# adjerbetian/OpenCL_PathTracer

Hardware: AMD Instinct MI355X
Metric: Msamples/s (paths x bounces) at 1920x1080 (higher is better)
Workload: dtype f32; 1 GPU; BASELINE configs[2]: synthetic random-triangle scene (numpy MT19937 seed 12345): 1000000 triangles (665533 BVH nodes, depth 22), 1920x1080, ray depth 10, JITTERED, 1 light(s); spp_total=256, parallelism=single GPU

## Files before the change

### opencl_pathtracer_amd/csrc/kernel_wavefront.hip

```cpp
#include <hip/hip_runtime.h>

#include "ptmi_device.hpp"
#include "ptmi_shading.hpp"
#include "ptmi_literal_path.hpp"

#include <atomic>
#include <cstdlib>
#include <cstring>

namespace PTMI_DEV_NS {

constexpr int kWfBlock = 256;
constexpr int kWfBlockNarrow = 64;
constexpr int kWfStack = PTMI_BVH_MAX_DEPTH;
#ifndef PTMI_WF_MIN_WAVES
#define PTMI_WF_MIN_WAVES 5
#endif
#ifndef PTMI_WF_MIN_WAVES_GENERAL
#define PTMI_WF_MIN_WAVES_GENERAL 5
#endif
#ifndef PTMI_WF_QUEUES
#define PTMI_WF_QUEUES 8
#endif
constexpr int kQueues = PTMI_WF_QUEUES;
// ... 20 lines not shown
    const DShade* shade;
    const DMat* mats;
    const ptmi_light* lights;
    const ptmi_texture* textures;
    const ptmi_uchar4* texels;
    uint32_t root_ref;
    uint32_t width, height;
    uint32_t max_depth, n_lights, sampler, tris_precomputed;
    uint32_t histograms;
    uint32_t boxes_ordered;
    uint32_t wide_records;
    uint32_t russian_roulette;
    uint32_t source_seed;
    uint32_t wait_debt;
    uint32_t split_paths;
};

constexpr uint32_t kStatDepthBins = 64;
constexpr uint32_t kPoisonMarker = 0x7FC0DEADu;
constexpr uint32_t kGivenUp = 0x80000000u, kGiveUpListFirst = (uint32_t)(kQueues * kQueueStride), kGiveUpListCap = 8u * 1024u - kGiveUpListFirst;
static_assert(kQueues * kQueueStride <= 1024, "the give-up list lies behind the queue counters inside the set's 8 x 1024 dwords");
constexpr uint32_t kSplitWords = C_TRI + 1;
static_assert(PTMI_COUNTER_SPLITS * (int)kSplitWords <= 64, "flushed by one wave");
__device__ __forceinline__ uint32_t counter_split_of(uint32_t slot, uint32_t split_paths)
{
    const uint32_t t1 = split_paths ? split_paths : 0xFFFFFFFFu, t2 = split_paths ? 2u * split_paths : 0xFFFFFFFFu,
                   t3 = split_paths ? 3u * split_paths : 0xFFFFFFFFu;
    return (slot >= t1 ? 1u : 0u) + (slot >= t2 ? 1u : 0u) + (slot >= t3 ? 1u : 0u);
}

// ... 24 lines not shown
    atomicAdd(&totals[C_SEGMENTS], (unsigned long long)n_seg - 1ull);
    atomicAdd(&totals[C_HITS], (unsigned long long)depth);
    atomicAdd(&totals[C_SHADOW], (unsigned long long)n_shadow);
    atomicAdd(&totals[C_BBX], (unsigned long long)pc.bbx);
    atomicAdd(&totals[C_TRI], (unsigned long long)pc.tri);
}

__device__ __forceinline__ void give_path_up(V4& radiance, V4& transfer, uint32_t& reflection, uint32_t& p_bbx, uint32_t& p_tri)
{
    const float m = __uint_as_float(kPoisonMarker);
    radiance = v4(m, m, m, m);
    transfer = v4(1, 1, 1, 1);
    reflection = 0; p_bbx = 0; p_tri = 0;
}

template <bool STATS, bool PRE, bool SS, bool PLAIN = false, bool NANSAFE = false, int BLOCK = 256>
__global__ void __launch_bounds__(BLOCK, PLAIN ? PTMI_WF_MIN_WAVES : PTMI_WF_MIN_WAVES_GENERAL) render_wavefront_kernel(
                                                                    const DScene* __restrict__ scene_in_memory, const DWarm sc_arg, const uint32_t first_iteration,
                                                                    const uint32_t n_iterations, const uint32_t iteration_stride,
                                                                    const uint32_t n_jobs,
                                                                    uint32_t* __restrict__ job_counter,
                                                                    const uint32_t stack_levels,
                                                                    float* __restrict__ stage,
                                                                    uint32_t* __restrict__ stage_stats)
{
    DWarm sc = sc_arg;
    if (PLAIN) { sc.sampler = PTMI_SAMPLER_JITTERED; sc.russian_roulette = 0; sc.n_lights = 1; }
    constexpr bool kOneLight = PLAIN;
    constexpr int kWfBlock = BLOCK;
    constexpr bool kTos = !PLAIN;
    extern __shared__ __attribute__((aligned(16))) uint32_t stack_mem[];
    constexpr uint32_t kBlockCounters = STATS ? (uint32_t)C_COUNT : PTMI_COUNTER_SPLITS * kSplitWords;
    static_assert(kBlockCounters <= 64, "zeroed and flushed by one wave");
    __shared__ unsigned long long block_counters[kBlockCounters];

    const uint32_t tid = threadIdx.x;
    if (tid < kBlockCounters) block_counters[tid] = 0;
    __syncthreads();
    uint32_t* const stack_floor = &stack_mem[kHitRecordWords * kWfBlock + tid];
    *stack_floor = REF_NONE;
    auto cold_scene = [&]() -> const DScene& {
        const DScene* p = scene_in_memory;
        asm volatile("" : "+s"(p));
        return *p;
    };
// ... 75 lines not shown
        cur = sc.root_ref; sp = stack_floor; tri_i = tri_end = 0;
        if (kTos) tos = REF_NONE;
        if (shadow) atomicAnd(&hit_mem[kWordTri * kWfBlock], ~kHitFound);
        else hit_mem[kWordTri * kWfBlock] = 0;
        exact_boxes = !(sc.boxes_ordered && ray_slabs_are_ordered(r));
        if (cur & REF_LEAF) {
            decode_leaf(sc, cur, tri_i, tri_end);
            cur = REF_NONE;
        }
    };

    unsigned long long* const key_mem = reinterpret_cast<unsigned long long*>(&stack_mem[(kHitRecordWords + 1 + stack_levels) * kWfBlock]);
    uint2* const item_mem = reinterpret_cast<uint2*>(&stack_mem[(kHitRecordWords + 3 + stack_levels) * kWfBlock]) + (tid & ~63u);
    const uint32_t lane = tid & 63u, wave_first = (uint32_t)__builtin_amdgcn_readfirstlane((int)(tid & ~63u));
    uint32_t pass_rounds = 0, pass_items = 0, item_violations = 0;
    const uint32_t n_records = STATS ? cold_scene().n_records : 0u;
    auto leaf_pass = [&](bool waits_at_leaf) {
        auto lanes_below = [&](unsigned long long m) {
            return __builtin_amdgcn_mbcnt_hi((uint32_t)(m >> 32), __builtin_amdgcn_mbcnt_lo((uint32_t)m, 0u));
        };
        const uint32_t left = tri_end - tri_i;
        const uint32_t offered = waits_at_leaf ? (left < 4u ? left : 4u) : 0u;
        const unsigned long long plane0 = __builtin_amdgcn_ballot_w64((offered & 1u) != 0), plane1 = __builtin_amdgcn_ballot_w64((offered & 2u) != 0),
                                 plane2 = __builtin_amdgcn_ballot_w64((offered & 4u) != 0);
        const int n_items = __popcll(plane0) + 2 * __popcll(plane1) + 4 * __popcll(plane2);
        const uint32_t first_item = lanes_below(plane0) + 2u * lanes_below(plane1) + 4u * lanes_below(plane2);
        const uint32_t room = first_item < 64u ? 64u - first_item : 0u;
        const uint32_t cnt = offered < room ? offered : room;
        const uint32_t n_now = n_items < 64 ? (uint32_t)n_items : 64u;
        if (STATS) { pass_rounds++; pass_items += n_now; }
// ... 63 lines not shown
                decode_leaf(sc, cur, tri_i, tri_end);
                cur = kTos ? tos : *sp;
                uint32_t* const under = sp - kWfBlock;
                sp = under < stack_floor ? stack_floor : under;
                if (kTos) tos = *sp;
            }
        }
    };
    auto node_step = [&]() {
        const float4* const rec = reinterpret_cast<const float4*>(&sc.tris[cur & REF_INDEX_MASK_INNER]);
        const float4 a = rec[0], b = rec[1], c = rec[2], d = rec[3];
        const float lo1[3] = {a.x, a.y, a.z}, hi1[3] = {a.w, b.x, b.y};
        const float lo2[3] = {b.z, b.w, c.x}, hi2[3] = {c.y, c.z, c.w};
        const uint32_t ref1 = __float_as_uint(d.x), ref2 = __float_as_uint(d.y), axis = __float_as_uint(d.z);
        const bool fwd = ((dir_signs >> axis) & 1u) != 0;
        bool h1, h2;
        if (!wave_exact) {
            h1 = box_hit_ordered(lo1, hi1, r, limit);
            h2 = box_hit_ordered(lo2, hi2, r, limit);
        } else {
            h1 = box_hit(lo1, hi1, (ref1 & REF_EMPTY) != 0, r, limit);
            h2 = box_hit(lo2, hi2, (ref2 & REF_EMPTY) != 0, r, limit);
        }
        p_bbx += 2;
        if (kTos) {
            const uint32_t far_ref = fwd ? ref2 : ref1;
            sp[kWfBlock] = far_ref;
            uint32_t* const pushed = sp + kWfBlock;
            const uint32_t child = fwd ? (h1 ? ref1 : ref2) : (h2 ? ref2 : ref1);
            cur = h1 ? child : (h2 ? child : tos);
            tos = h1 ? (h2 ? far_ref : tos) : tos;
            sp = h1 ? (h2 ? pushed : sp) : sp;
            if (!(h1 | h2)) {
                uint32_t* const below = sp - kWfBlock;
                sp = below < stack_floor ? stack_floor : below;
                tos = *sp;
            }
            if (cur != REF_NONE && (cur & REF_LEAF)) {
                decode_leaf(sc, cur, tri_i, tri_end);
                cur = tos;
                uint32_t* const under = sp - kWfBlock;
                sp = under < stack_floor ? stack_floor : under;
                tos = *sp;
            }
            return;
        }
        sp[kWfBlock] = fwd ? ref2 : ref1;
        uint32_t* const pushed = sp + kWfBlock;
        sp = h1 ? (h2 ? pushed : sp) : sp;
        const uint32_t popped = *sp;
        uint32_t* const below = sp - kWfBlock;
        uint32_t* const under = below < stack_floor ? stack_floor : below;
        const uint32_t child = fwd ? (h1 ? ref1 : ref2) : (h2 ? ref2 : ref1);
        cur = h1 ? child : (h2 ? child : popped);
        sp = h1 ? sp : (h2 ? sp : under);
        if (cur != REF_NONE && (cur & REF_LEAF)) {
            decode_leaf(sc, cur, tri_i, tri_end);
            cur = *sp;
            uint32_t* const under = sp - kWfBlock;
            sp = under < stack_floor ? stack_floor : under;
        }
    };

    int wait_debt = 0;
    bool pending, want_inner, want_post;
    int n_t, n_i, n_p;
    bool any_lane;
    unsigned long long dead_lanes = 0ull;
    auto survey = [&]() {
        pending = tri_i < tri_end;
        const bool has_node = cur < REF_DEAD;
        const unsigned long long b_t = __builtin_amdgcn_ballot_w64(pending), b_n = __builtin_amdgcn_ballot_w64(has_node), b_dead = dead_lanes;
        const unsigned long long m_t = b_t, m_i = b_n & ~b_t, m_p = ~(b_t | b_n | b_dead);
        want_inner = !pending & has_node;
        want_post = !pending & !has_node & (cur != REF_DEAD);
// ... 175 lines not shown
                }
                if (skip) {
                    if (owns_pixel) cold_scene().stage_flag[gy * sc.width + gx] = 0.f;
                    need_path = true;
                } else
                if (sc.max_depth > 0) {
                    limit = INFINITY;
                    new_ray = true;
                } else {
                    finish_path(false);
                }
            }
            if (new_ray) {
                ray_set_direction(r, new_direction);
                dir_signs = (r.d.x > 0 ? 1u : 0u) | (r.d.y > 0 ? 2u : 0u) | (r.d.z > 0 ? 4u : 0u);
                const float o_size = __builtin_fabsf(r.o.x) + __builtin_fabsf(r.o.y) + __builtin_fabsf(r.o.z) + __builtin_fabsf(r.o.w);
                const float d_size = __builtin_fabsf(r.d.x) + __builtin_fabsf(r.d.y) + __builtin_fabsf(r.d.z) + __builtin_fabsf(r.d.w);
                bool bad = !((o_size <= 0x1p+40f) & (d_size <= 4.0f));
                if (!PLAIN && !owns_pixel && __builtin_expect(bad, 0)) {
                    const uint32_t place = atomicAdd(&job_counter[2], 1u);
                    bad = place < kGiveUpListCap;
                    if (bad) {
                        job_counter[kGiveUpListFirst + place] = slot;
                        slot |= kGivenUp;
                    }
                }
                if (__builtin_expect(bad, 0)) {
                    give_path_up(radiance, transfer, reflection, p_bbx, p_tri);
                    shadow = false;
                    job_counter[1] = 1u;
// ... 6 lines not shown
        dead_lanes = __builtin_amdgcn_ballot_w64(cur == REF_DEAD);
        wave_exact = __builtin_amdgcn_ballot_w64(exact_boxes) != 0ull;
        if (STATS) cycles_p += __builtin_amdgcn_s_memtime() - pass_start;
    }

    if (STATS && (tid & 63u) == 0) {
        atomicAdd(&block_counters[C_TRIPS_I], (unsigned long long)trips_i);
        atomicAdd(&block_counters[C_LANES_I], lanes_i);
        atomicAdd(&block_counters[C_TRIPS_T], (unsigned long long)(pass_rounds));
        atomicAdd(&block_counters[C_LANES_T], (unsigned long long)pass_items);
        atomicAdd(&block_counters[C_TRIPS_P], (unsigned long long)trips_p);
        atomicAdd(&block_counters[C_LANES_P], lanes_p);
        atomicAdd(&block_counters[C_CYCLES_P], cycles_p);
        atomicAdd(&block_counters[C_CYCLES_LOOP], __builtin_amdgcn_s_memtime() - loop_start);
    }
    if (STATS && item_violations != 0u) atomicAdd(&block_counters[C_ITEM_VIOLATIONS], (unsigned long long)item_violations);
    __syncthreads();
    if (tid < (STATS ? 1u : (uint32_t)PTMI_COUNTER_SPLITS)) {
        unsigned long long* const totals = &block_counters[tid * kSplitWords];
        totals[C_SHADOW] = totals[C_HITS] * sc.n_lights;
    }
    __syncthreads();
    if (STATS) {
        if (tid < C_COUNT) atomicAdd(&cold_scene().counters[tid], block_counters[tid]);
    } else if (tid < kBlockCounters) {
        const uint32_t k = tid / kSplitWords, c = tid % kSplitWords;
        if (k == 0u || block_counters[tid] != 0ull) atomicAdd(&cold_scene().counters[k * C_COUNT + c], block_counters[tid]);
    }
}

// ... 235 lines not shown

static bool five_wide_workgroups_fit(const WavefrontLaunch& w)
{
    static std::atomic<int> wide_fits[kMaxCachedDevices][PTMI_BVH_MAX_DEPTH + 1];
    int fits = w.cached_device ? wide_fits[w.device][w.lv].load(std::memory_order_relaxed) : 0;
    if (fits == 0) {
        int n_cu = 0;
        const int wide = resident_blocks_of(PTMI_DEV_NS::render_wavefront_kernel<false, true, false, true, false>, w.lv, PTMI_DEV_NS::kWfBlock);
        const bool known = hipDeviceGetAttribute(&n_cu, hipDeviceAttributeMultiprocessorCount, w.device) == hipSuccess && n_cu > 0 && wide > 0;
        fits = known && wide < 5 * n_cu ? 2 : 1;
        if (w.cached_device) wide_fits[w.device][w.lv].store(fits, std::memory_order_relaxed);
    }
    return fits == 1;
}

template <bool S, bool P, bool A, bool L, bool N, int B>
static void launch_instance(const WavefrontLaunch& w)
{
    auto kernel = PTMI_DEV_NS::render_wavefront_kernel<S, P, A, L, N, B>;
    static std::atomic<int> resident_cache[kMaxCachedDevices][PTMI_BVH_MAX_DEPTH + 1];
    int resident = w.cached_device ? resident_cache[w.device][w.lv].load(std::memory_order_relaxed) : 0;
    if (resident == 0) {
        resident = resident_blocks_of(kernel, w.lv, B);
        if (w.cached_device) resident_cache[w.device][w.lv].store(resident, std::memory_order_relaxed);
    }
    if (w.cached_device) g_last_grid[w.device].store((uint32_t)B << 20 | (uint32_t)resident, std::memory_order_relaxed);
    uint32_t nb = (w.n_jobs + B - 1) / B;
    if (resident > 0 && nb > (uint32_t)resident) nb = (uint32_t)resident;
    hipLaunchKernelGGL(kernel, dim3(nb), dim3(B), wavefront_lds_bytes(w.lv, B), w.st, w.scene_in_device_memory, w.warm, w.first_iteration,
                       w.n_iterations, w.iteration_stride, w.n_jobs, w.job_counter, w.lv, w.stage, w.stage_stats);
}

using LaunchInstance = void (*)(const WavefrontLaunch&);
static LaunchInstance instance_for(const DScene& sc, bool scheduler_stats, bool plain, bool narrow)
{
    constexpr int kWide = PTMI_DEV_NS::kWfBlock, kNarrow = PTMI_DEV_NS::kWfBlockNarrow;
    const bool pre = sc.tris_precomputed != 0;
    if (sc.super_sampling) return pre ? launch_instance<true, true, true, false, true, kWide> : launch_instance<true, false, true, false, true, kWide>;
    if (scheduler_stats) return pre ? launch_instance<true, true, false, false, true, kWide> : launch_instance<true, false, false, false, true, kWide>;
    if (sc.nan_safe) {
        if (plain) return launch_instance<false, true, false, true, true, kWide>;
        return pre ? launch_instance<false, true, false, false, true, kWide> : launch_instance<false, false, false, false, true, kWide>;
    }
    if (plain)
        return narrow ? launch_instance<false, true, false, true, false, kNarrow> : launch_instance<false, true, false, true, false, kWide>;
    if (pre) return narrow ? launch_instance<false, true, false, false, false, kNarrow> : launch_instance<false, true, false, false, false, kWide>;
    return launch_instance<false, false, false, false, false, kWide>;
}

}

int PTMI_ARITH(launch_render_wavefront)(const DScene& sc, const DScene* scene_in_device_memory, uint32_t first_iteration,
                            uint32_t n_iterations, uint32_t iteration_stride, uint32_t* job_counter, uint32_t stack_levels,
                            bool scheduler_stats, float* stage, uint32_t* stage_stats, void* stream, std::string* err)
{
    if (n_iterations == 0) return PTMI_OK;
    const uint32_t tiles = ((sc.width + 7u) / 8u) * ((sc.height + 7u) / 8u);
    const uint64_t jobs64 = (uint64_t)tiles * 64u * n_iterations;
    if (jobs64 > (sc.sampler == PTMI_SAMPLER_RANDOM ? 0x7FFFFFF0ull : 0xFFFFFFF0ull)) {
        if (err) *err = "too many jobs in one launch";
        return PTMI_ERR_INVALID_ARGUMENT;
// ... 12 lines not shown
        w.first_iteration = first_iteration; w.n_iterations = n_iterations; w.iteration_stride = iteration_stride;
        w.job_counter = job_counter; w.stage = stage; w.stage_stats = stage_stats;
        w.cached_device = hipGetDevice(&w.device) == hipSuccess && w.device >= 0 && w.device < kMaxCachedDevices;
        const uint32_t lv = w.lv;
        PTMI_DEV_NS::DWarm& warm = w.warm;
        warm.nodes = sc.nodes; warm.tris = sc.tris; warm.big_leaves = sc.big_leaves; warm.tri_ids = sc.tri_ids; warm.shade = sc.shade;
        warm.mats = sc.mats; warm.lights = sc.lights; warm.textures = sc.textures; warm.texels = sc.texels;
        warm.root_ref = sc.root_ref; warm.width = sc.width; warm.height = sc.height; warm.max_depth = sc.max_depth;
        warm.n_lights = sc.n_lights; warm.sampler = sc.sampler; warm.tris_precomputed = sc.tris_precomputed;
        warm.histograms = sc.hist_depths != nullptr;
        warm.boxes_ordered = sc.boxes_ordered;
        warm.wide_records = sc.wide_records;
        warm.russian_roulette = sc.russian_roulette;
        warm.source_seed = sc.source_seed;
        warm.split_paths = sc.split_paths;
        const bool plain = sc.tris_precomputed && sc.plain_shading && sc.sampler == PTMI_SAMPLER_JITTERED && !sc.russian_roulette &&
                           sc.n_lights == 1 && !sc.super_sampling && !scheduler_stats;
        warm.wait_debt = lv >= 16u ? 768u : (plain ? 320u : 512u);
        const bool narrow = !five_wide_workgroups_fit(w) && std::getenv("PTMI_WIDE_WORKGROUPS") == nullptr;
        instance_for(sc, scheduler_stats, plain, narrow)(w);
        e = hipGetLastError();
        const dim3 redo_block(PTMI_DEV_NS::kBlock);
        if (e == hipSuccess && stage == nullptr && sc.sampler == PTMI_SAMPLER_RANDOM) {
            const auto redo_random = sc.tris_precomputed ? PTMI_DEV_NS::redo_random_kernel<true> : PTMI_DEV_NS::redo_random_kernel<false>;
            hipLaunchKernelGGL(redo_random, dim3(64), redo_block, 0, w.st, sc, first_iteration, n_iterations, iteration_stride, job_counter);
            e = hipGetLastError();
        }
        if (e == hipSuccess && stage != nullptr) {
            const auto redo_poisoned = sc.tris_precomputed ? PTMI_DEV_NS::redo_poisoned_kernel<true> : PTMI_DEV_NS::redo_poisoned_kernel<false>;
            hipLaunchKernelGGL(redo_poisoned, dim3(1024), redo_block, 0, w.st, sc, first_iteration, n_iterations, iteration_stride, stage,
// ... 36 lines not shown
```

### opencl_pathtracer_amd/csrc/ptmi_api.cpp

```cpp
#include <cstdlib>
#include <cstring>
#include <mutex>

#include "ptmi_context.h"

using namespace ptmi_internal;

namespace {
std::mutex g_err_mutex;
std::string g_err;
}

void ptmi_internal::set_global_error(const std::string& msg)
{
    std::lock_guard<std::mutex> lock(g_err_mutex);
    g_err = msg;
}

extern "C" {

int ptmi_abi_version(void) { return PTMI_ABI_VERSION; }

int ptmi_device_count(void)
{
// ... 57 lines not shown
        return fail(nullptr, PTMI_ERR_HIP, msg);
    }
    {
        const uint64_t tiles = (uint64_t)((cfg->image_width + 7u) / 8u) * ((cfg->image_height + 7u) / 8u);
        const uint64_t by_jobs = (cfg->sampler == PTMI_SAMPLER_RANDOM ? 0x7FFFFFF0ull : 0xFFFFFFF0ull) / (tiles * 64u);
        const uint64_t by_bytes = (4ull << 30) / ((uint64_t)cfg->image_width * cfg->image_height * 20u);
        uint64_t cap = kMaxIterationsPerLaunch;
        if (by_jobs < cap) cap = by_jobs;
        if (by_bytes < cap) cap = by_bytes;
        ctx->iterations_per_launch = cap < 1 ? 1u : (uint32_t)cap;
        if (const char* v = std::getenv("PTMI_ITERATIONS_PER_LAUNCH")) {
            const long want = std::strtol(v, nullptr, 10);
            if (want >= 1 && want <= 32 && (uint32_t)want < ctx->iterations_per_launch) ctx->iterations_per_launch = (uint32_t)want;
        }
    }
    *out = ctx;
    return PTMI_OK;
}

int ptmi_set_stream(ptmi_ctx* ctx, void* hip_stream)
{
    if (!ctx) return PTMI_ERR_INVALID_ARGUMENT;
    if (ctx->n_dev() != 1) return fail(ctx, PTMI_ERR_UNSUPPORTED, "ptmi_set_stream on a multi-device context");
    DeviceState& d = ctx->dev[0];
    ON_DEVICE(ctx, d);
    HIP_TRY(ctx, hipStreamSynchronize(d.stream));
    if (int rc = fold_events(ctx, d)) return rc;
    d.stream = hip_stream ? (hipStream_t)hip_stream : d.own_stream;
    return PTMI_OK;
}
// ... 186 lines not shown
```

### opencl_pathtracer_amd/csrc/ptmi_context.h

```cpp
#pragma once

#include <hip/hip_runtime.h>

#include <string>
#include <utility>
#include <vector>

#include "ptmi.h"
#include "ptmi_internal.h"
#include "scene_refit.h"
#include "launch_schedule.h"
#include "snapshot_ring.h"

namespace ptmi_internal {

struct DeviceScene {
    std::vector<void*> allocations;
    float* d_color = nullptr;
    float* d_count = nullptr;
    uint32_t* d_hist = nullptr;
    unsigned long long* d_counters = nullptr;
    uint32_t* d_job_counter = nullptr;
    DScene ds{};
    DScene* d_scene = nullptr;
// ... 36 lines not shown
    UpdateFacts update;
    RefitSchedule refit;
    bool have_refit = false;
    float* d_reduced = nullptr;
    uint8_t* d_display = nullptr;
    size_t display_bytes = 0;
};

}

struct ptmi_ctx : ptmi_internal::ContextScene {
    ptmi_config cfg{};
    std::vector<ptmi_internal::DeviceState> dev;
    std::string err;
    uint32_t iterations_per_launch = ptmi_internal::kMaxIterationsPerLaunch;
    std::vector<void*> rccl_comms;
    int rccl_state = 0;
    float* h_staging = nullptr;
    struct HostRange { char* p; size_t bytes; };
    std::vector<HostRange> pinned_host;
    char* d_query = nullptr;
    char* h_query = nullptr;
    size_t query_cap = 0;

    ptmi_internal::ContextScene& scene() { return *this; }
    uint32_t n_dev() const { return (uint32_t)dev.size(); }
    size_t npix() const { return (size_t)cfg.image_width * cfg.image_height; }
    size_t color_bytes() const { return npix() * 16; }
    size_t count_bytes() const { return npix() * 4; }
    size_t image_bytes() const { return npix() * 20; }
// ... 72 lines not shown
```

### opencl_pathtracer_amd/csrc/ptmi_internal.h

```cpp
#pragma once

#include <cstdint>
#include <string>

#include "ptmi.h"
#ifdef __HIPCC__
#include <hip/hip_runtime.h>
#endif

namespace ptmi_internal {

void set_global_error(const std::string& msg);

#ifdef __HIPCC__
inline int launch_status(hipError_t e, const char* kernel, std::string* err)
{
    if (e == hipSuccess) return PTMI_OK;
    if (err) *err = std::string(kernel) + " launch: " + hipGetErrorString(e);
    return PTMI_ERR_HIP;
}
#endif

constexpr uint32_t REF_LEAF = 0x80000000u;
constexpr uint32_t REF_EMPTY = 0x40000000u;
// ... 89 lines not shown
    uint32_t root_ref;
    uint32_t width, height;
    uint32_t max_depth;
    uint32_t n_lights;
    uint32_t sampler;
    uint32_t super_sampling;
    uint32_t tris_precomputed;
    uint32_t plain_shading;
    uint32_t nan_safe;
    uint32_t nan_walk_box_tests, nan_walk_tri_tests, nan_walk_last_tri;
    uint32_t n_records;
    uint32_t wide_records;
    uint32_t boxes_ordered;
    uint32_t russian_roulette;
    uint32_t source_seed;
};

#define PTMI_DECLARE_INTEGRATOR_ENTRY_POINTS(SUFFIX)                                                                             \
                                       \
    int launch_render##SUFFIX(const DScene& sc, uint32_t first_iteration, uint32_t n_iterations, uint32_t iteration_stride,      \
                              void* stream, std::string* err);                                                                  \
                            \
      \
    int launch_render_wavefront##SUFFIX(const DScene& sc, const DScene* scene_in_device_memory, uint32_t first_iteration,        \
                                        uint32_t n_iterations, uint32_t iteration_stride, uint32_t* job_counter,                \
                                        uint32_t stack_levels, bool scheduler_stats, float* stage,                              \
                                        uint32_t* stage_stats, void* stream, std::string* err);                                 \
    void last_wavefront_grid##SUFFIX(int device, uint32_t* lanes_per_workgroup, uint32_t* resident_workgroups);                  \
           \
    int launch_accumulate_staged##SUFFIX(const DScene& sc, uint32_t first_iteration, uint32_t n_iterations, const float* stage,  \
// ... 26 lines not shown
```

### opencl_pathtracer_amd/csrc/ptmi_scene_memory.cpp

```cpp
#include <algorithm>
#include <chrono>
#include <cstdlib>
#include <cstring>

#include "ptmi_context.h"
#include "scene_layout.h"

using namespace ptmi_internal;

bool ptmi_internal::one_path_per_lane(const ptmi_ctx* ctx)
{
    if ((ctx->cfg.flags & PTMI_FLAG_MEGAKERNEL) != 0) return true;
    if (ctx->literal_kernel_reason.empty()) return false;
    const char* force = std::getenv("PTMI_LITERAL_KERNEL");
    return ctx->cfg.sampler == PTMI_SAMPLER_RANDOM || (force && force[0] == '1');
}

int ptmi_internal::quiesce(ptmi_ctx* ctx, DeviceState& d)
{
    ON_DEVICE(ctx, d);
    d.schedule.forget();
    for (int i = 0; i < kStageSets; i++)
        if (d.launch_stream[i]) HIP_TRY(ctx, hipStreamSynchronize(d.launch_stream[i]));
    HIP_TRY(ctx, hipStreamSynchronize(d.stream));
// ... 128 lines not shown
        if (int rc = scene_alloc(ctx, d, ctx->count_bytes(), ds.stage_flag)) return rc;
        HIP_TRY(ctx, hipMemcpy(dx, kX2inv, sizeof kX2inv, hipMemcpyHostToDevice));
        ds.x2inv = dx;
    }
    ds.sky = *sc->sky;
    std::memcpy(ds.cam_pos, &sc->camera_position, 16);
    std::memcpy(ds.cam_dir, &sc->camera_direction, 16);
    std::memcpy(ds.cam_right, &sc->camera_right, 16);
    std::memcpy(ds.cam_up, &sc->camera_up, 16);
    ds.tris_precomputed = lay.tris_precomputed ? 1u : 0u;
    ds.plain_shading = lay.plain_shading ? 1u : 0u;
    ds.nan_safe = lay.literal_kernel_reason.empty() ? 0u : 1u;
    ds.nan_walk_box_tests = lay.nan_walk_box_tests; ds.nan_walk_tri_tests = lay.nan_walk_tri_tests; ds.nan_walk_last_tri = lay.nan_walk_last_tri;
    if (std::getenv("PTMI_WALK_NAN_RAYS") != nullptr) ds.nan_walk_box_tests = ds.nan_walk_tri_tests = 0xFFFFFFFFu;
    ds.boxes_ordered = (lay.boxes_ordered && std::getenv("PTMI_GENERIC_BOXES") == nullptr) ? 1u : 0u;
    ds.root_ref = lay.root_ref;
    ds.width = ctx->cfg.image_width;
    ds.height = ctx->cfg.image_height;
    ds.max_depth = ctx->cfg.ray_max_depth;
    ds.n_lights = ctx->cfg.lights_size;
    ds.sampler = ctx->cfg.sampler;
    ds.russian_roulette = (ctx->cfg.flags & PTMI_FLAG_RUSSIAN_ROULETTE) ? 1u : 0u;
    ds.source_seed = (ctx->cfg.flags & PTMI_FLAG_SOURCE_SEED) ? 1u : 0u;
    return upload_scene_records(ctx, d);
}

}

extern "C" {

// ... 254 lines not shown
```

### opencl_pathtracer_amd/csrc/scene_layout.cpp

```cpp
#include "scene_layout.h"
#include "scene_refit_common.h"

#include <cmath>
#include <cstdlib>
#include <cstring>
#include <limits>

namespace ptmi_internal {

namespace {

int fail(std::string& err, int code, const std::string& msg)
{
    err = msg;
    return code;
}



bool texture_ok(const ptmi_texture& t, uint32_t data_size)
{
    if (t.width == 0 || t.height == 0) return false;
    const uint64_t end = (uint64_t)t.offset + (uint64_t)t.width * t.height;
    return end <= data_size;
// ... 104 lines not shown
        const ptmi_triangle& t = sc->triangulation[i];
        if (int rc = check_triangle_materials(t, i, out.material_is_simple_color.data(), sc->materiaux_size, err)) return rc;
        ptmi_refit::make_tri_record(t, &out.tris[i]);
        ptmi_refit::make_shade_record(t, &out.shade[i]);
    }

    out.literal_kernel_reason = scene_needs_literal_kernel(sc);

    out.tris_precomputed = std::getenv("PTMI_GENERIC_TRIANGLES") == nullptr;
    for (uint32_t i = 0; i < nt && out.tris_precomputed; i++)
        if (!ptmi_refit::triangle_keeps_equal_w(sc->triangulation[i])) out.tris_precomputed = false;
    if (out.tris_precomputed)
        for (uint32_t i = 0; i < nt; i++)
            ptmi_refit::make_tri_record_pre(sc->triangulation[i], reinterpret_cast<DTriPre*>(&out.tris[i]));

    std::vector<uint8_t> seen(nn, 0);
    std::string why;
    auto check_node = [&](uint32_t id) -> bool {
        if (id >= nn) { why = "child index out of range"; return false; }
        if (seen[id]) { why = "node " + std::to_string(id) + " reached twice (cycle or shared subtree)"; return false; }
        seen[id] = 1;
        const ptmi_node& n = sc->bvh[id];
        if (n.is_leaf) {
            if ((uint64_t)n.triangle_start_index + n.nb_triangles > nt) { why = "leaf triangle range out of bounds"; return false; }
        } else if (n.cut_axis > 2) { why = "cutAxis > 2"; return false; }
        return true;
    };
    auto emit_leaf = [&](uint32_t id, uint32_t* ref) -> bool {
        const ptmi_node& n = sc->bvh[id];
        const size_t start = out.recs.size();
// ... 37 lines not shown
        if (!check_node(n.son1_id) || !check_node(n.son2_id))
            return fail(err, PTMI_ERR_BAD_SCENE, "bvh[" + std::to_string(it.id) + "]: " + why);
        const ptmi_node& c1 = sc->bvh[n.son1_id];
        const ptmi_node& c2 = sc->bvh[n.son2_id];
        uint32_t r1 = c1.triangles_aabb.is_empty ? REF_EMPTY : 0u, r2 = c2.triangles_aabb.is_empty ? REF_EMPTY : 0u;
        if (c1.is_leaf && !emit_leaf(n.son1_id, &r1)) return fail(err, PTMI_ERR_LIMIT, "bvh[" + std::to_string(it.id) + "]: " + why);
        if (c2.is_leaf && !emit_leaf(n.son2_id, &r2)) return fail(err, PTMI_ERR_LIMIT, "bvh[" + std::to_string(it.id) + "]: " + why);
        DNode& d = node_at(self);
        const ptmi_bounding_box& b1 = c1.triangles_aabb;
        const ptmi_bounding_box& b2 = c2.triangles_aabb;
        d.lo1[0] = b1.p_min.x; d.lo1[1] = b1.p_min.y; d.lo1[2] = b1.p_min.z;
        d.hi1[0] = b1.p_max.x; d.hi1[1] = b1.p_max.y; d.hi1[2] = b1.p_max.z;
        d.lo2[0] = b2.p_min.x; d.lo2[1] = b2.p_min.y; d.lo2[2] = b2.p_min.z;
        d.hi2[0] = b2.p_max.x; d.hi2[1] = b2.p_max.y; d.hi2[2] = b2.p_max.z;
        d.ref1 = r1; d.ref2 = r2; d.axis = n.cut_axis; d.pad = 0;
        for (int k = 0; k < 3; k++) {
            if (!(r1 & REF_EMPTY) && !(std::isfinite(d.lo1[k]) && std::isfinite(d.hi1[k]) && d.lo1[k] <= d.hi1[k])) out.boxes_ordered = false;
            if (!(r2 & REF_EMPTY) && !(std::isfinite(d.lo2[k]) && std::isfinite(d.hi2[k]) && d.lo2[k] <= d.hi2[k])) out.boxes_ordered = false;
        }
        const uint32_t child_depth = it.depth + 1;
        if (child_depth > out.max_depth) out.max_depth = child_depth;
        if (!c2.is_leaf) todo.push_back({n.son2_id, (uint32_t)self, 1, child_depth});
        if (!c1.is_leaf) todo.push_back({n.son1_id, (uint32_t)self, 0, child_depth});
    }
    if (out.recs.empty()) { out.recs.emplace_back(); out.tri_ids.push_back(0xFFFFFFFFu); }
    if (out.boxes_ordered)
        for (size_t i = 0; i < out.recs.size(); i++) {
            if (out.tri_ids[i] != 0xFFFFFFFFu) continue;
            DNode& d = node_at(i);
            const float inf = std::numeric_limits<float>::infinity();
// ... 62 lines not shown
```

### opencl_pathtracer_amd/csrc/scene_layout.h

```cpp
#pragma once

#include <string>
#include <vector>

#include "ptmi.h"
#include "ptmi_internal.h"

namespace ptmi_internal {

struct Relayout {
    std::vector<DTri> recs;
    std::vector<uint32_t> tri_ids;
    std::vector<DTri> tris;
    std::vector<DShade> shade;
    std::vector<DMat> mats;
    std::vector<uint8_t> material_is_simple_color;
    std::vector<DBigLeaf> big_leaves;
    bool tris_precomputed = false;
    bool plain_shading = false;
    bool boxes_ordered = true;
    std::string literal_kernel_reason;
    uint32_t root_ref = 0;
    uint32_t max_depth = 0;
    uint32_t nan_walk_box_tests = 0, nan_walk_tri_tests = 0, nan_walk_last_tri = 0xFFFFFFFFu;
};

std::string camera_needs_literal_kernel(const ptmi_float4& position, const ptmi_float4& direction, const ptmi_float4& right, const ptmi_float4& up);
std::string triangle_needs_literal_kernel(const ptmi_triangle& t, uint32_t i);
int check_triangle_materials(const ptmi_triangle& t, uint32_t i, const uint8_t* material_is_simple_color, uint32_t materiaux_size, std::string& err);

int build_layout(const ptmi_config& cfg, const ptmi_scene* sc, Relayout& out, std::string& err);

}
```

### opencl_pathtracer_amd/csrc/scene_refit_common.h

```cpp
#ifndef PTMI_SCENE_REFIT_COMMON_H
#define PTMI_SCENE_REFIT_COMMON_H

#include <cmath>
#include <cstdint>

#include "bvh_build_common.h"
#include "ptmi_internal.h"

namespace ptmi_refit {

using ptmi_bvh::PBox;
using ptmi_internal::DBigLeaf;
using ptmi_internal::DNode;
using ptmi_internal::DShade;
using ptmi_internal::DTri;
using ptmi_internal::DTriPre;

PTMI_HD float dot4(const float a[4], const float b[4])
{
    return fmaf(a[3], b[3], fmaf(a[2], b[2], fmaf(a[1], b[1], a[0] * b[0])));
}

PTMI_HD void triangle_edges(const ptmi_triangle& t, float u[4], float v[4])
{
// ... 78 lines not shown
        }
    } else {
        const DNode& c = nodes[ref & REF_INDEX_MASK_INNER];
        const PBox first = (c.ref1 & REF_EMPTY) ? ptmi_bvh::pbox_empty() : corners_box(c.lo1, c.hi1);
        const PBox second = (c.ref2 & REF_EMPTY) ? ptmi_bvh::pbox_empty() : corners_box(c.lo2, c.hi2);
        b = ptmi_bvh::pbox_merge(first, second);
    }
    lo[0] = keep_sel(lo[0], b.p_min.x); lo[1] = keep_sel(lo[1], b.p_min.y); lo[2] = keep_sel(lo[2], b.p_min.z);
    hi[0] = keep_sel(hi[0], b.p_max.x); hi[1] = keep_sel(hi[1], b.p_max.y); hi[2] = keep_sel(hi[2], b.p_max.z);
}

PTMI_HD void refit_record(DNode* d, const DNode* nodes, const DBigLeaf* big_leaves, const uint32_t* tri_ids, const ptmi_triangle* tris)
{
    if (!(d->ref1 & ptmi_internal::REF_EMPTY)) refit_child_box(d->ref1, nodes, big_leaves, tri_ids, tris, d->lo1, d->hi1);
    if (!(d->ref2 & ptmi_internal::REF_EMPTY)) refit_child_box(d->ref2, nodes, big_leaves, tri_ids, tris, d->lo2, d->hi2);
}

}

#endif
```

Measured before the change: 972.5 Msamples/s.

## Skip certified BVH leaves whose box lies beyond the current hit distance

Adds a leaf-culling pass. When the scene layout is built, each BVH record gets per-child bits that mark leaves whose triangles pass a numeric-slack certification. During traversal the kernel computes the squared distance from the ray origin to each child box. It then skips decoding a certified leaf when that distance exceeds the current hit limit plus a tolerance, and counts the skipped triangle tests. New template instances are selected when culling is enabled, either by environment variable or automatically when enough leaves certify. The cost is extra ALU work and register pressure in every box test, and the pruning may rarely apply because the slab test already bounds entry distance.

```diff
diff --git a/opencl_pathtracer_amd/csrc/kernel_wavefront.hip b/opencl_pathtracer_amd/csrc/kernel_wavefront.hip
--- a/opencl_pathtracer_amd/csrc/kernel_wavefront.hip
+++ b/opencl_pathtracer_amd/csrc/kernel_wavefront.hip
@@ -1,5 +1,6 @@
 #include <hip/hip_runtime.h>
 
+#include "leaf_cull.h"
 #include "ptmi_device.hpp"
 #include "ptmi_shading.hpp"
 #include "ptmi_literal_path.hpp"
@@ -58,6 +59,7 @@
     uint32_t source_seed;
     uint32_t wait_debt;
     uint32_t split_paths;
+    uint32_t leaf_cull;
 };
 
 constexpr uint32_t kStatDepthBins = 64;
@@ -112,7 +114,7 @@
     reflection = 0; p_bbx = 0; p_tri = 0;
 }
 
-template <bool STATS, bool PRE, bool SS, bool PLAIN = false, bool NANSAFE = false, int BLOCK = 256>
+template <bool STATS, bool PRE, bool SS, bool PLAIN = false, bool NANSAFE = false, int BLOCK = 256, bool CULL = false>
 __global__ void __launch_bounds__(BLOCK, PLAIN ? PTMI_WF_MIN_WAVES : PTMI_WF_MIN_WAVES_GENERAL) render_wavefront_kernel(
                                                                     const DScene* __restrict__ scene_in_memory, const DWarm sc_arg, const uint32_t first_iteration,
                                                                     const uint32_t n_iterations, const uint32_t iteration_stride,
@@ -127,6 +129,8 @@
     constexpr bool kOneLight = PLAIN;
     constexpr int kWfBlock = BLOCK;
     constexpr bool kTos = !PLAIN;
+    static_assert(!CULL || PRE, "cull bits are computed for precomputed records only");
+    constexpr bool kCull = CULL;
     extern __shared__ __attribute__((aligned(16))) uint32_t stack_mem[];
     constexpr uint32_t kBlockCounters = STATS ? (uint32_t)C_COUNT : PTMI_COUNTER_SPLITS * kSplitWords;
     static_assert(kBlockCounters <= 64, "zeroed and flushed by one wave");
@@ -232,6 +236,7 @@
     uint2* const item_mem = reinterpret_cast<uint2*>(&stack_mem[(kHitRecordWords + 3 + stack_levels) * kWfBlock]) + (tid & ~63u);
     const uint32_t lane = tid & 63u, wave_first = (uint32_t)__builtin_amdgcn_readfirstlane((int)(tid & ~63u));
     uint32_t pass_rounds = 0, pass_items = 0, item_violations = 0;
+    uint32_t culled_items = 0;
     const uint32_t n_records = STATS ? cold_scene().n_records : 0u;
     auto leaf_pass = [&](bool waits_at_leaf) {
         auto lanes_below = [&](unsigned long long m) {
@@ -325,6 +330,12 @@
         const float lo2[3] = {b.z, b.w, c.x}, hi2[3] = {c.y, c.z, c.w};
         const uint32_t ref1 = __float_as_uint(d.x), ref2 = __float_as_uint(d.y), axis = __float_as_uint(d.z);
         const bool fwd = ((dir_signs >> axis) & 1u) != 0;
+        float d2_1 = 0, d2_2 = 0;
+        if (kCull) {
+            d2_1 = ptmi_cull::box_distance2(lo1, hi1, r.o.x, r.o.y, r.o.z);
+            d2_2 = ptmi_cull::box_distance2(lo2, hi2, r.o.x, r.o.y, r.o.z);
+            asm volatile("" : "+v"(d2_1), "+v"(d2_2));
+        }
         bool h1, h2;
         if (!wave_exact) {
             h1 = box_hit_ordered(lo1, hi1, r, limit);
@@ -334,6 +345,13 @@
             h2 = box_hit(lo2, hi2, (ref2 & REF_EMPTY) != 0, r, limit);
         }
         p_bbx += 2;
+        bool culled = false;
+        if (kCull) {
+            const uint32_t cull_bits = __float_as_uint(d.w) & (dir_signs >> 3) & sc.leaf_cull;
+            const bool first = fwd ? h1 : !h2;
+            const bool certified = (cull_bits & (first ? ptmi_cull::kCullChild1 : ptmi_cull::kCullChild2)) != 0u;
+            culled = (h1 | h2) & certified & ptmi_cull::box_is_beyond(first ? d2_1 : d2_2, limit);
+        }
         if (kTos) {
             const uint32_t far_ref = fwd ? ref2 : ref1;
             sp[kWfBlock] = far_ref;
@@ -348,11 +366,23 @@
                 tos = *sp;
             }
             if (cur != REF_NONE && (cur & REF_LEAF)) {
-                decode_leaf(sc, cur, tri_i, tri_end);
-                cur = tos;
-                uint32_t* const under = sp - kWfBlock;
-                sp = under < stack_floor ? stack_floor : under;
-                tos = *sp;
+                bool leaf = true;
+                if (kCull && culled) {
+                    p_tri += (cur >> REF_COUNT_SHIFT) & 7u;
+                    if (STATS) culled_items += (cur >> REF_COUNT_SHIFT) & 7u;
+                    cur = tos;
+                    uint32_t* const under = sp - kWfBlock;
+                    sp = under < stack_floor ? stack_floor : under;
+                    tos = *sp;
+                    leaf = cur != REF_NONE && (cur & REF_LEAF);
+                }
+                if (leaf) {
+                    decode_leaf(sc, cur, tri_i, tri_end);
+                    cur = tos;
+                    uint32_t* const under = sp - kWfBlock;
+                    sp = under < stack_floor ? stack_floor : under;
+                    tos = *sp;
+                }
             }
             return;
         }
@@ -366,10 +396,21 @@
         cur = h1 ? child : (h2 ? child : popped);
         sp = h1 ? sp : (h2 ? sp : under);
         if (cur != REF_NONE && (cur & REF_LEAF)) {
-            decode_leaf(sc, cur, tri_i, tri_end);
-            cur = *sp;
-            uint32_t* const under = sp - kWfBlock;
-            sp = under < stack_floor ? stack_floor : under;
+            bool leaf = true;
+            if (kCull && culled) {
+                p_tri += (cur >> REF_COUNT_SHIFT) & 7u;
+                if (STATS) culled_items += (cur >> REF_COUNT_SHIFT) & 7u;
+                cur = *sp;
+                uint32_t* const under = sp - kWfBlock;
+                sp = under < stack_floor ? stack_floor : under;
+                leaf = cur != REF_NONE && (cur & REF_LEAF);
+            }
+            if (leaf) {
+                decode_leaf(sc, cur, tri_i, tri_end);
+                cur = *sp;
+                uint32_t* const under = sp - kWfBlock;
+                sp = under < stack_floor ? stack_floor : under;
+            }
         }
     };
 
@@ -575,6 +616,7 @@
             if (new_ray) {
                 ray_set_direction(r, new_direction);
                 dir_signs = (r.d.x > 0 ? 1u : 0u) | (r.d.y > 0 ? 2u : 0u) | (r.d.z > 0 ? 4u : 0u);
+                if (kCull && ptmi_cull::ray_may_cull(r.o.x, r.o.y, r.o.z, r.o.w, r.d.w)) dir_signs |= (ptmi_cull::kCullChild1 | ptmi_cull::kCullChild2) << 3;
                 const float o_size = __builtin_fabsf(r.o.x) + __builtin_fabsf(r.o.y) + __builtin_fabsf(r.o.z) + __builtin_fabsf(r.o.w);
                 const float d_size = __builtin_fabsf(r.d.x) + __builtin_fabsf(r.d.y) + __builtin_fabsf(r.d.z) + __builtin_fabsf(r.d.w);
                 bool bad = !((o_size <= 0x1p+40f) & (d_size <= 4.0f));
@@ -611,6 +653,7 @@
         atomicAdd(&block_counters[C_CYCLES_P], cycles_p);
         atomicAdd(&block_counters[C_CYCLES_LOOP], __builtin_amdgcn_s_memtime() - loop_start);
     }
+    if (STATS && culled_items != 0u) atomicAdd(&block_counters[C_LANES_T], (unsigned long long)culled_items);
     if (STATS && item_violations != 0u) atomicAdd(&block_counters[C_ITEM_VIOLATIONS], (unsigned long long)item_violations);
     __syncthreads();
     if (tid < (STATS ? 1u : (uint32_t)PTMI_COUNTER_SPLITS)) {
@@ -876,10 +919,10 @@
     return fits == 1;
 }
 
-template <bool S, bool P, bool A, bool L, bool N, int B>
+template <bool S, bool P, bool A, bool L, bool N, int B, bool C = false>
 static void launch_instance(const WavefrontLaunch& w)
 {
-    auto kernel = PTMI_DEV_NS::render_wavefront_kernel<S, P, A, L, N, B>;
+    auto kernel = PTMI_DEV_NS::render_wavefront_kernel<S, P, A, L, N, B, C>;
     static std::atomic<int> resident_cache[kMaxCachedDevices][PTMI_BVH_MAX_DEPTH + 1];
     int resident = w.cached_device ? resident_cache[w.device][w.lv].load(std::memory_order_relaxed) : 0;
     if (resident == 0) {
@@ -898,15 +941,21 @@
 {
     constexpr int kWide = PTMI_DEV_NS::kWfBlock, kNarrow = PTMI_DEV_NS::kWfBlockNarrow;
     const bool pre = sc.tris_precomputed != 0;
-    if (sc.super_sampling) return pre ? launch_instance<true, true, true, false, true, kWide> : launch_instance<true, false, true, false, true, kWide>;
-    if (scheduler_stats) return pre ? launch_instance<true, true, false, false, true, kWide> : launch_instance<true, false, false, false, true, kWide>;
+    const bool cull = pre && sc.leaf_cull != 0u;
+    if (sc.super_sampling) return pre ? launch_instance<true, true, true, false, true, kWide, true> : launch_instance<true, false, true, false, true, kWide>;
+    if (scheduler_stats) return pre ? launch_instance<true, true, false, false, true, kWide, true> : launch_instance<true, false, false, false, true, kWide>;
     if (sc.nan_safe) {
         if (plain) return launch_instance<false, true, false, true, true, kWide>;
         return pre ? launch_instance<false, true, false, false, true, kWide> : launch_instance<false, false, false, false, true, kWide>;
     }
-    if (plain)
+    if (plain) {
+        if (cull) return narrow ? launch_instance<false, true, false, true, false, kNarrow, true> : launch_instance<false, true, false, true, false, kWide, true>;
         return narrow ? launch_instance<false, true, false, true, false, kNarrow> : launch_instance<false, true, false, true, false, kWide>;
-    if (pre) return narrow ? launch_instance<false, true, false, false, false, kNarrow> : launch_instance<false, true, false, false, false, kWide>;
+    }
+    if (pre) {
+        if (cull) return narrow ? launch_instance<false, true, false, false, false, kNarrow, true> : launch_instance<false, true, false, false, false, kWide, true>;
+        return narrow ? launch_instance<false, true, false, false, false, kNarrow> : launch_instance<false, true, false, false, false, kWide>;
+    }
     return launch_instance<false, false, false, false, false, kWide>;
 }
 
@@ -949,6 +998,7 @@
         warm.russian_roulette = sc.russian_roulette;
         warm.source_seed = sc.source_seed;
         warm.split_paths = sc.split_paths;
+        warm.leaf_cull = sc.leaf_cull;
         const bool plain = sc.tris_precomputed && sc.plain_shading && sc.sampler == PTMI_SAMPLER_JITTERED && !sc.russian_roulette &&
                            sc.n_lights == 1 && !sc.super_sampling && !scheduler_stats;
         warm.wait_debt = lv >= 16u ? 768u : (plain ? 320u : 512u);
diff --git a/opencl_pathtracer_amd/csrc/leaf_cull.h b/opencl_pathtracer_amd/csrc/leaf_cull.h
--- /dev/null
+++ b/opencl_pathtracer_amd/csrc/leaf_cull.h
@@ -0,0 +1,127 @@
+#ifndef PTMI_LEAF_CULL_H
+#define PTMI_LEAF_CULL_H
+
+#include <cmath>
+#include <cstdint>
+
+#include "ptmi_internal.h"
+
+#if defined(__HIPCC__)
+#include <hip/hip_runtime.h>
+#define PTMI_CULL_HD __host__ __device__ __forceinline__
+#else
+#define PTMI_CULL_HD inline
+#endif
+
+namespace ptmi_cull {
+
+constexpr float kRel = 1.001f, kAbs = 0.01f, kMaxOrigin = 0x1p+41f;
+constexpr double kKappaMax = 0x1p-13, kEpsAbsMax = 2.0e-3;
+
+constexpr uint32_t kCullChild1 = 1u, kCullChild2 = 2u, kCullComputed = 4u;
+
+PTMI_CULL_HD float box_distance2(const float lo[3], const float hi[3], float ox, float oy, float oz)
+{
+    const float dx = fmaxf(fmaxf(lo[0] - ox, ox - hi[0]), 0.0f);
+    const float dy = fmaxf(fmaxf(lo[1] - oy, oy - hi[1]), 0.0f);
+    const float dz = fmaxf(fmaxf(lo[2] - oz, oz - hi[2]), 0.0f);
+    return fmaf(dz, dz, fmaf(dy, dy, dx * dx));
+}
+
+PTMI_CULL_HD bool ray_may_cull(float ox, float oy, float oz, float ow, float dw)
+{
+    return fabsf(ox) + fabsf(oy) + fabsf(oz) <= kMaxOrigin && ow == 1.0f && dw == 0.0f;
+}
+PTMI_CULL_HD bool box_is_beyond(float d2, float limit)
+{
+    return d2 > fmaf(limit, kRel, kAbs);
+}
+PTMI_CULL_HD bool leaf_cull_rule(float d2, float limit, float ox, float oy, float oz, float ow, float dw)
+{
+    return box_is_beyond(d2, limit) && ray_may_cull(ox, oy, oz, ow, dw);
+}
+
+PTMI_CULL_HD bool triangle_slack(const ptmi_triangle& t, const float lo[3], const float hi[3], double* eps_abs, double* kappa)
+{
+    const double u24 = 0x1p-24;
+    const float S[3][3] = {{t.s1.x, t.s1.y, t.s1.z}, {t.s2.x, t.s2.y, t.s2.z}, {t.s3.x, t.s3.y, t.s3.z}};
+    if (!(t.s1.w == t.s2.w && t.s1.w == t.s3.w && fabsf(t.s1.w) <= 0x1p+20f)) return false;
+    if (!(t.n.w == 0.0f || (t.s1.w == 1.0f && fabsf(t.n.w) <= 4.0f))) return false;
+    double B2 = 0;
+    for (int k = 0; k < 3; k++) {
+        if (!(lo[k] <= hi[k] && fabsf(lo[k]) <= 0x1p+20f && fabsf(hi[k]) <= 0x1p+20f)) return false;
+        for (int j = 0; j < 3; j++)
+            if (!(S[j][k] >= lo[k] && S[j][k] <= hi[k])) return false;
+        const double m = fmax(fabs((double)lo[k]), fabs((double)hi[k]));
+        B2 += m * m;
+    }
+    const double B = sqrt(B2);
+    const float uf[3] = {S[1][0] - S[0][0], S[1][1] - S[0][1], S[1][2] - S[0][2]}, vf[3] = {S[2][0] - S[0][0], S[2][1] - S[0][1], S[2][2] - S[0][2]};
+    const float uv_c = fmaf(uf[2], vf[2], fmaf(uf[1], vf[1], uf[0] * vf[0])), uu_c = fmaf(uf[2], uf[2], fmaf(uf[1], uf[1], uf[0] * uf[0])),
+                vv_c = fmaf(vf[2], vf[2], fmaf(vf[1], vf[1], vf[0] * vf[0]));
+    const double ud[3] = {uf[0], uf[1], uf[2]}, vd[3] = {vf[0], vf[1], vf[2]};
+    const double uu = ud[0] * ud[0] + ud[1] * ud[1] + ud[2] * ud[2], vv = vd[0] * vd[0] + vd[1] * vd[1] + vd[2] * vd[2],
+                 uv = ud[0] * vd[0] + ud[1] * vd[1] + ud[2] * vd[2];
+    const double lu = sqrt(uu), lv = sqrt(vv);
+    if (!(lu >= 0x1p-16 && lv >= 0x1p-16)) return false;
+    const double cr[3] = {ud[1] * vd[2] - ud[2] * vd[1], ud[2] * vd[0] - ud[0] * vd[2], ud[0] * vd[1] - ud[1] * vd[0]};
+    const double area2 = sqrt(cr[0] * cr[0] + cr[1] * cr[1] + cr[2] * cr[2]);
+    if (!(area2 > 0)) return false;
+    const double N[3] = {t.n.x, t.n.y, t.n.z};
+    const double Nn = (N[0] * cr[0] + N[1] * cr[1] + N[2] * cr[2]) / area2, len_n = sqrt(N[0] * N[0] + N[1] * N[1] + N[2] * N[2]);
+    if (!(fabs(Nn) >= 0.25 && len_n <= 4.0)) return false;
+    const double tan2 = len_n * len_n - Nn * Nn;
+    const double tilt = sqrt(tan2 > 0 ? tan2 : 0) / fabs(Nn);
+    if (!(tilt <= 0x1p-18)) return false;
+    const float det_c[2] = {uv_c * uv_c - uu_c * vv_c, fmaf(uv_c, uv_c, -(uu_c * vv_c))};
+    double dk = 0, c_w = 0;
+    for (int m = 0; m < 2; m++) {
+        if (!(det_c[m] < 0.0f)) return false;
+        const double den = (double)(1.0f / det_c[m]);
+        if (!std::isfinite(den)) return false;
+        const double k11 = den * ((double)uv_c * uv - (double)vv_c * uu) - 1.0, k12 = den * ((double)uv_c * vv - (double)vv_c * uv);
+        const double k21 = den * ((double)uv_c * uu - (double)uu_c * uv), k22 = den * ((double)uv_c * uv - (double)uu_c * vv) - 1.0;
+        dk = fmax(dk, fmax(fabs(k11) + fabs(k12), fabs(k21) + fabs(k22)) + 8 * u24);
+        const double e = 10.1 * u24 * fabs(den) * (1 + 8 * u24), es = e * lu * lv * lv, et = e * lu * lu * lv;
+        const double ss = es + 0.025 * (es + et), st = et + 0.025 * (es + et);
+        c_w = fmax(c_w, fmax(ss * lu + st * lv, fmax((ss + 2 * st) * lu + st * lv, ss * lu + (2 * ss + st) * lv)));
+    }
+    if (!(dk <= 0.01)) return false;
+    const double diam = sqrt(((double)hi[0] - lo[0]) * ((double)hi[0] - lo[0]) + ((double)hi[1] - lo[1]) * ((double)hi[1] - lo[1]) +
+                             ((double)hi[2] - lo[2]) * ((double)hi[2] - lo[2]));
+    *kappa = 0x1p-18 + 2 * c_w;
+    *eps_abs = 32 * u24 * (B + fabs((double)t.n.w) / fabs(Nn)) + c_w * diam + (5 * dk + 4 * u24 + 2 * tilt) * (lu + lv);
+    return std::isfinite(*kappa) && std::isfinite(*eps_abs);
+}
+
+PTMI_CULL_HD bool triangle_certified(const ptmi_triangle& t, const float lo[3], const float hi[3])
+{
+    double eps_abs, kappa;
+    return triangle_slack(t, lo, hi, &eps_abs, &kappa) && eps_abs <= kEpsAbsMax && kappa <= kKappaMax;
+}
+
+template <class TriAt>
+PTMI_CULL_HD bool leaf_is_cullable(uint32_t ref, const float lo[3], const float hi[3], TriAt tri_at)
+{
+    using namespace ptmi_internal;
+    if (!(ref & REF_LEAF) || (ref & REF_EMPTY)) return false;
+    const uint32_t count = (ref >> REF_COUNT_SHIFT) & 7u;
+    if (count == 0u || count == REF_COUNT_BIG) return false;
+    for (uint32_t k = 0; k < count; k++)
+        if (!triangle_certified(tri_at(k), lo, hi)) return false;
+    return true;
+}
+
+template <class TriOfRecord>
+PTMI_CULL_HD uint32_t record_cull_bits(const ptmi_internal::DNode& d, TriOfRecord tri_of_record)
+{
+    const uint32_t start1 = d.ref1 & ptmi_internal::REF_INDEX_MASK_LEAF, start2 = d.ref2 & ptmi_internal::REF_INDEX_MASK_LEAF;
+    uint32_t bits = kCullComputed;
+    if (leaf_is_cullable(d.ref1, d.lo1, d.hi1, [&](uint32_t k) -> const ptmi_triangle& { return tri_of_record(start1 + k); })) bits |= kCullChild1;
+    if (leaf_is_cullable(d.ref2, d.lo2, d.hi2, [&](uint32_t k) -> const ptmi_triangle& { return tri_of_record(start2 + k); })) bits |= kCullChild2;
+    return bits;
+}
+
+}
+
+#endif
diff --git a/opencl_pathtracer_amd/csrc/ptmi_api.cpp b/opencl_pathtracer_amd/csrc/ptmi_api.cpp
--- a/opencl_pathtracer_amd/csrc/ptmi_api.cpp
+++ b/opencl_pathtracer_amd/csrc/ptmi_api.cpp
@@ -95,6 +95,7 @@
             if (want >= 1 && want <= 32 && (uint32_t)want < ctx->iterations_per_launch) ctx->iterations_per_launch = (uint32_t)want;
         }
     }
+    if (const char* v = std::getenv("PTMI_LEAF_CULL")) ctx->leaf_cull = v[0] != '0' ? 1 : 0;
     *out = ctx;
     return PTMI_OK;
 }
diff --git a/opencl_pathtracer_amd/csrc/ptmi_context.h b/opencl_pathtracer_amd/csrc/ptmi_context.h
--- a/opencl_pathtracer_amd/csrc/ptmi_context.h
+++ b/opencl_pathtracer_amd/csrc/ptmi_context.h
@@ -74,6 +74,7 @@
     std::vector<ptmi_internal::DeviceState> dev;
     std::string err;
     uint32_t iterations_per_launch = ptmi_internal::kMaxIterationsPerLaunch;
+    int leaf_cull = -1;
     std::vector<void*> rccl_comms;
     int rccl_state = 0;
     float* h_staging = nullptr;
diff --git a/opencl_pathtracer_amd/csrc/ptmi_internal.h b/opencl_pathtracer_amd/csrc/ptmi_internal.h
--- a/opencl_pathtracer_amd/csrc/ptmi_internal.h
+++ b/opencl_pathtracer_amd/csrc/ptmi_internal.h
@@ -127,6 +127,7 @@
     uint32_t boxes_ordered;
     uint32_t russian_roulette;
     uint32_t source_seed;
+    uint32_t leaf_cull;
 };
 
 #define PTMI_DECLARE_INTEGRATOR_ENTRY_POINTS(SUFFIX)                                                                             \
diff --git a/opencl_pathtracer_amd/csrc/ptmi_scene_memory.cpp b/opencl_pathtracer_amd/csrc/ptmi_scene_memory.cpp
--- a/opencl_pathtracer_amd/csrc/ptmi_scene_memory.cpp
+++ b/opencl_pathtracer_amd/csrc/ptmi_scene_memory.cpp
@@ -3,6 +3,7 @@
 #include <cstdlib>
 #include <cstring>
 
+#include "leaf_cull.h"
 #include "ptmi_context.h"
 #include "scene_layout.h"
 
@@ -166,6 +167,10 @@
     ds.nan_walk_box_tests = lay.nan_walk_box_tests; ds.nan_walk_tri_tests = lay.nan_walk_tri_tests; ds.nan_walk_last_tri = lay.nan_walk_last_tri;
     if (std::getenv("PTMI_WALK_NAN_RAYS") != nullptr) ds.nan_walk_box_tests = ds.nan_walk_tri_tests = 0xFFFFFFFFu;
     ds.boxes_ordered = (lay.boxes_ordered && std::getenv("PTMI_GENERIC_BOXES") == nullptr) ? 1u : 0u;
+    constexpr uint32_t kCullMinLeaves = 1024;
+    const bool cull_bits = lay.tris_precomputed && lay.literal_kernel_reason.empty();
+    const bool cull = ctx->leaf_cull < 0 ? lay.cullable_leaves >= kCullMinLeaves : ctx->leaf_cull != 0;
+    ds.leaf_cull = (cull && cull_bits) ? (ptmi_cull::kCullChild1 | ptmi_cull::kCullChild2) : 0u;
     ds.root_ref = lay.root_ref;
     ds.width = ctx->cfg.image_width;
     ds.height = ctx->cfg.image_height;
diff --git a/opencl_pathtracer_amd/csrc/scene_layout.cpp b/opencl_pathtracer_amd/csrc/scene_layout.cpp
--- a/opencl_pathtracer_amd/csrc/scene_layout.cpp
+++ b/opencl_pathtracer_amd/csrc/scene_layout.cpp
@@ -142,6 +142,7 @@
         for (uint32_t i = 0; i < nt; i++)
             ptmi_refit::make_tri_record_pre(sc->triangulation[i], reinterpret_cast<DTriPre*>(&out.tris[i]));
 
+    const bool cull_bits = out.tris_precomputed && out.literal_kernel_reason.empty();
     std::vector<uint8_t> seen(nn, 0);
     std::string why;
     auto check_node = [&](uint32_t id) -> bool {
@@ -209,6 +210,8 @@
         d.lo2[0] = b2.p_min.x; d.lo2[1] = b2.p_min.y; d.lo2[2] = b2.p_min.z;
         d.hi2[0] = b2.p_max.x; d.hi2[1] = b2.p_max.y; d.hi2[2] = b2.p_max.z;
         d.ref1 = r1; d.ref2 = r2; d.axis = n.cut_axis; d.pad = 0;
+        if (cull_bits) d.pad = ptmi_cull::record_cull_bits(d, [&](uint32_t r) -> const ptmi_triangle& { return sc->triangulation[out.tri_ids[r]]; });
+        out.cullable_leaves += ((d.pad & ptmi_cull::kCullChild1) ? 1u : 0u) + ((d.pad & ptmi_cull::kCullChild2) ? 1u : 0u);
         for (int k = 0; k < 3; k++) {
             if (!(r1 & REF_EMPTY) && !(std::isfinite(d.lo1[k]) && std::isfinite(d.hi1[k]) && d.lo1[k] <= d.hi1[k])) out.boxes_ordered = false;
             if (!(r2 & REF_EMPTY) && !(std::isfinite(d.lo2[k]) && std::isfinite(d.hi2[k]) && d.lo2[k] <= d.hi2[k])) out.boxes_ordered = false;
diff --git a/opencl_pathtracer_amd/csrc/scene_layout.h b/opencl_pathtracer_amd/csrc/scene_layout.h
--- a/opencl_pathtracer_amd/csrc/scene_layout.h
+++ b/opencl_pathtracer_amd/csrc/scene_layout.h
@@ -19,6 +19,7 @@
     bool tris_precomputed = false;
     bool plain_shading = false;
     bool boxes_ordered = true;
+    uint32_t cullable_leaves = 0;
     std::string literal_kernel_reason;
     uint32_t root_ref = 0;
     uint32_t max_depth = 0;
diff --git a/opencl_pathtracer_amd/csrc/scene_refit_common.h b/opencl_pathtracer_amd/csrc/scene_refit_common.h
--- a/opencl_pathtracer_amd/csrc/scene_refit_common.h
+++ b/opencl_pathtracer_amd/csrc/scene_refit_common.h
@@ -5,6 +5,7 @@
 #include <cstdint>
 
 #include "bvh_build_common.h"
+#include "leaf_cull.h"
 #include "ptmi_internal.h"
 
 namespace ptmi_refit {
@@ -116,6 +117,8 @@
 {
     if (!(d->ref1 & ptmi_internal::REF_EMPTY)) refit_child_box(d->ref1, nodes, big_leaves, tri_ids, tris, d->lo1, d->hi1);
     if (!(d->ref2 & ptmi_internal::REF_EMPTY)) refit_child_box(d->ref2, nodes, big_leaves, tri_ids, tris, d->lo2, d->hi2);
+    if (d->pad & ptmi_cull::kCullComputed)
+        d->pad = ptmi_cull::record_cull_bits(*d, [&](uint32_t r) -> const ptmi_triangle& { return tris[tri_ids[r]]; });
 }
 
 }
```

After: 1004 Msamples/s, median of 6. 3.3% higher.
